# ChenFengYe/motion-latent-diffusion

Hardware: NVIDIA H100
Metric: motions/sec @ 50-step DDIM text-to-motion, batch 256 (higher is better)
Workload: dtype f16x2-split (fp32-equivalent, fp32 accumulate)

## Files before the change

include/mldb.h:

```cpp
#ifndef MLDB_H_
#define MLDB_H_

#include <stdint.h>

#ifdef __cplusplus
extern "C" {
#endif

#define MLDB_OK 0
#define MLDB_ERR_INVALID 1
#define MLDB_ERR_CUDA 2
#define MLDB_ERR_STATE 3
#define MLDB_ERR_UNSUPPORTED 4

#define MLDB_ABI_VERSION 4

typedef struct mldb_handle mldb_handle;

#define MLDB_COND_TEXT 0
#define MLDB_COND_ACTION 1
#define MLDB_ARCH_TRANS_ENC 0
#define MLDB_ARCH_TRANS_DEC 1
#define MLDB_VAE_NONE 0
#define MLDB_VAE_MLD 1
// ... 75 lines not shown

int mldb_feats2joints(mldb_handle* h, const float* feats, int32_t B, int32_t T,
                      float* joints_out, void* stream);

int mldb_sample(mldb_handle* h, const void* cond, const float* init_noise,
                const int32_t* lengths, int32_t B, int32_t S_ctx, int32_t T,
                float* latents_out, float* feats_out, float* joints_out, void* stream,
                const float* step_noise);

int mldb_sample_host(mldb_handle* h, const void* cond_host, const float* init_noise_host,
                     const int32_t* lengths_host, int32_t B, int32_t S_ctx, int32_t T,
                     float* joints_host, void* stream, const float* step_noise_host);

int mldb_comm_unique_id(void* out128 );
int mldb_comm_init(mldb_handle* h, const void* unique_id128, int32_t nranks, int32_t rank);
int mldb_comm_attach(mldb_handle* h, void* nccl_comm, int32_t nranks, int32_t rank);
int mldb_comm_info(const mldb_handle* h, int32_t* nranks, int32_t* rank);
int mldb_allgather(mldb_handle* h, const float* local, float* global, int64_t count, void* stream);
int mldb_sample_gather(mldb_handle* h, const void* cond, const float* init_noise, const int32_t* lengths,
                       int32_t B, int32_t S_ctx, int32_t T, float* joints_global, void* stream,
                       const float* step_noise);
int mldb_gather_wait(mldb_handle* h, void* stream);

int mldb_profile_op(mldb_handle* h, const char* op, int32_t B, int32_t S_ctx, int32_t iters,
                    float* avg_ms_out);

int mldb_profile_steps(mldb_handle* h, const void* cond, const float* init_noise, int32_t B, int32_t S_ctx,
                       float* ms_out);

int mldb_debug_timeline(int32_t enable, int64_t* out, int32_t cap, int32_t* count);

int mldb_debug_gemm(mldb_handle* h, const float* A, const float* W, const float* bias, const float* gamma,
                    const float* beta, const float* R, int32_t M, int32_t N, int32_t K, int32_t K1,
                    int32_t act, int32_t use_tc, int32_t split_out, float* out, void* stream);

int mldb_debug_ffn(mldb_handle* h, const float* X, const float* W1, const float* b1, const float* W2,
                   const float* b2, const float* gamma, const float* beta, int32_t M, int32_t d, int32_t ff,
                   int32_t mode, float* out, void* stream);

int mldb_debug_tail(mldb_handle* h, const float* att, const float* X, const float* Wo, const float* bo,
                    const float* gamma1, const float* beta1, const float* W1, const float* b1, const float* W2,
                    const float* b2, const float* gamma2, const float* beta2, int32_t M, int32_t d, int32_t ff,
                    int32_t mode, int32_t out_rows, float* out, void* stream);

int mldb_debug_attention(mldb_handle* h, const float* Q, const float* KV, const int32_t* lengths, int32_t kv_prefix,
                         int32_t nseq, int32_t Lq, int32_t Lk, int32_t heads, int32_t hd, int32_t mode, float* out,
                         void* stream);

int mldb_debug_attention_causal(mldb_handle* h, const float* Q, const float* KV, const int32_t* lengths,
                                int32_t kv_prefix, int32_t nseq, int32_t Lq, int32_t Lk, int32_t heads, int32_t hd,
                                int32_t mode, float* out, void* stream);

#define MLDB_TEXT_ABI_VERSION 1
#define MLDB_TEXT_HIDDEN 0
#define MLDB_TEXT_POOLED 1
typedef struct mldb_text_config {
  int32_t abi_version;
  int32_t vocab_size;
  int32_t max_positions;
  int32_t hidden;
  int32_t heads;
  int32_t layers;
  int32_t ff;
  int32_t projection_dim;
  int32_t eos_token_id;
  float   ln_eps;
} mldb_text_config;
// ... 55 lines not shown
```

mld_b200/_lib.py:

```python
from __future__ import annotations

import ctypes as C
import os

_HERE = os.path.dirname(os.path.abspath(__file__))
LIB_PATH = os.path.join(_HERE, "libmldb200.so")

MLDB_ABI_VERSION = 4
COND_TEXT, COND_ACTION = 0, 1
ARCH_TRANS_ENC, ARCH_TRANS_DEC = 0, 1
VAE_NONE, VAE_MLD, VAE_ACTOR = 0, 1, 2
SCHED_DDIM, SCHED_DDPM = 0, 1
BETA_SCHEDULES = {"scaled_linear": 0, "linear": 1, "squaredcos_cap_v2": 2}
DTYPE_F32 = 0
KSTAT_NAMES = ("gemm_tc", "gemm_ln_tc", "ffn_tc", "attn_tc", "attn_mma", "attn_simt", "gemm_simt", "ln_simt",
               "ln_unfused", "misc", "text_ln", "gru_tc")
MLDB_TEXT_ABI_VERSION = 1
TEXT_HIDDEN, TEXT_POOLED = 0, 1
MLDB_T2M_ABI_VERSION = 1
T2M_TEXT, T2M_MOVEMENT, T2M_MOTION = 1, 2, 4


class MldbConfig(C.Structure):
    _fields_ = [
# ... 22 lines not shown

class MldbT2mConfig(C.Structure):
    _fields_ = [
        ("abi_version", C.c_int32), ("parts", C.c_int32), ("dim_word", C.c_int32), ("dim_pos_ohot", C.c_int32),
        ("dim_text_hidden", C.c_int32), ("dim_coemb_hidden", C.c_int32), ("dim_pose", C.c_int32),
        ("dim_move_hidden", C.c_int32), ("dim_move_latent", C.c_int32), ("dim_motion_hidden", C.c_int32),
        ("dim_motion_latent", C.c_int32),
    ]


_P = C.c_void_p
_SIGNATURES = {
    "mldb_default_config": (None, [C.POINTER(MldbConfig)]),
    "mldb_create": (C.c_int, [C.POINTER(MldbConfig), C.c_int, C.POINTER(_P)]),
    "mldb_destroy": (None, [_P]),
    "mldb_load_tensor": (C.c_int, [_P, C.c_char_p, _P, C.POINTER(C.c_int64), C.c_int32, C.c_int32]),
    "mldb_finalize_weights": (C.c_int, [_P, _P]),
    "mldb_set_mean_std": (C.c_int, [_P, _P, _P, C.c_int32]),
    "mldb_scheduler_table": (C.c_int, [C.POINTER(MldbConfig), _P]),
    "mldb_scheduler_timesteps": (C.c_int, [C.POINTER(MldbConfig), C.c_int32, _P]),
    "mldb_scheduler_set_timesteps": (C.c_int, [_P, C.c_int32, _P]),
    "mldb_scheduler_step": (C.c_int, [_P, _P, C.c_int64, _P, _P, C.c_int64, _P, _P]),
    "mldb_denoise": (C.c_int, [_P, _P, C.c_int64, _P, _P, C.c_int32, C.c_int32, C.c_int32, _P, _P]),
    "mldb_diffusion_reverse": (C.c_int, [_P, _P, _P, _P, _P, C.c_int32, C.c_int32, C.c_int32, _P, _P]),
    "mldb_vae_decode": (C.c_int, [_P, _P, _P, C.c_int32, C.c_int32, _P, _P]),
    "mldb_vae_encode": (C.c_int, [_P, _P, _P, C.c_int32, C.c_int32, _P, _P, _P]),
    "mldb_feats2joints": (C.c_int, [_P, _P, C.c_int32, C.c_int32, _P, _P]),
    "mldb_sample": (C.c_int, [_P, _P, _P, _P, C.c_int32, C.c_int32, C.c_int32, _P, _P, _P, _P, _P]),
    "mldb_sample_host": (C.c_int, [_P, _P, _P, _P, C.c_int32, C.c_int32, C.c_int32, _P, _P, _P]),
    "mldb_profile_op": (C.c_int, [_P, C.c_char_p, C.c_int32, C.c_int32, C.c_int32, C.POINTER(C.c_float)]),
    "mldb_profile_steps": (C.c_int, [_P, _P, _P, C.c_int32, C.c_int32, _P]),
    "mldb_debug_timeline": (C.c_int, [C.c_int32, _P, C.c_int32, C.POINTER(C.c_int32)]),
    "mldb_debug_gemm": (C.c_int, [_P, _P, _P, _P, _P, _P, _P, C.c_int32, C.c_int32, C.c_int32, C.c_int32,
                                  C.c_int32, C.c_int32, C.c_int32, _P, _P]),
    "mldb_debug_ffn": (C.c_int, [_P, _P, _P, _P, _P, _P, _P, _P, C.c_int32, C.c_int32, C.c_int32, C.c_int32, _P, _P]),
    "mldb_debug_tail": (C.c_int, [_P] * 13 + [C.c_int32] * 5 + [_P, _P]),
    "mldb_debug_attention": (C.c_int, [_P, _P, _P, _P, C.c_int32, C.c_int32, C.c_int32, C.c_int32, C.c_int32, C.c_int32,
                                       C.c_int32, _P, _P]),
    "mldb_debug_attention_causal": (C.c_int, [_P, _P, _P, _P, C.c_int32, C.c_int32, C.c_int32, C.c_int32, C.c_int32,
                                              C.c_int32, C.c_int32, _P, _P]),
    "mldb_default_text_config": (None, [C.POINTER(MldbTextConfig)]),
    "mldb_text_configure": (C.c_int, [_P, C.POINTER(MldbTextConfig)]),
    "mldb_text_encode": (C.c_int, [_P, _P, C.c_int32, C.c_int32, C.c_int32, _P, _P]),
    "mldb_default_t2m_config": (None, [C.POINTER(MldbT2mConfig)]),
    "mldb_t2m_configure": (C.c_int, [_P, C.POINTER(MldbT2mConfig)]),
    "mldb_t2m_movement": (C.c_int, [_P, _P, C.c_int32, C.c_int32, C.c_int32, _P, _P]),
    "mldb_t2m_motion": (C.c_int, [_P, _P, _P, C.c_int32, C.c_int32, _P, _P]),
    "mldb_t2m_text": (C.c_int, [_P, _P, _P, _P, C.c_int32, C.c_int32, _P, _P]),
    "mldb_comm_unique_id": (C.c_int, [_P]),
    "mldb_comm_init": (C.c_int, [_P, _P, C.c_int32, C.c_int32]),
    "mldb_comm_attach": (C.c_int, [_P, _P, C.c_int32, C.c_int32]),
    "mldb_comm_info": (C.c_int, [_P, C.POINTER(C.c_int32), C.POINTER(C.c_int32)]),
    "mldb_allgather": (C.c_int, [_P, _P, _P, C.c_int64, _P]),
    "mldb_sample_gather": (C.c_int, [_P, _P, _P, _P, C.c_int32, C.c_int32, C.c_int32, _P, _P, _P]),
    "mldb_gather_wait": (C.c_int, [_P, _P]),
    "mldb_kernel_stats": (C.c_int, [_P, _P, C.c_int32]),
    "mldb_reset_kernel_stats": (C.c_int, [_P]),
    "mldb_last_error": (C.c_char_p, []),
    "mldb_abi_version": (C.c_int, []),
    "mldb_launch_count": (C.c_int64, [_P]),
    "mldb_set_option": (C.c_int, [_P, C.c_char_p, C.c_char_p]),
}

_lib = None


def lib():
# ... 40 lines not shown
```

mld_b200/csrc/engine.cu:

```cuda
#include "engine.h"

#include <math.h>
#include <stdio.h>
#include <string.h>

#include <algorithm>

#include "gemm_tc.h"

static thread_local std::string g_err;
void mldb_set_err(const std::string& s) { g_err = s; }
extern "C" const char* mldb_last_error(void) { return g_err.c_str(); }
extern "C" int mldb_abi_version(void) { return MLDB_ABI_VERSION; }

#define CK(call)                                                                      \
  do {                                                                                \
    cudaError_t e__ = (call);                                                         \
    if (e__ != cudaSuccess) {                                                         \
      char buf__[512];                                                                \
      snprintf(buf__, sizeof buf__, "%s:%d: %s failed: %s", __FILE__, __LINE__, #call, \
               cudaGetErrorString(e__));                                              \
      mldb_set_err(buf__);                                                            \
      return MLDB_ERR_CUDA;                                                           \
    }                                                                                 \
// ... 2119 lines not shown
  TRY(t2m_ready(h, MLDB_T2M_TEXT, "text"));
  const mldb_t2m_config& c = h->t2m.cfg;
  if (B < 1 || L < 1 || (int64_t)B * L > (1 << 26)) FAIL(MLDB_ERR_INVALID, "text encoder input must be [B >= 1, L >= 1, *], got B=%d L=%d", B, L);
  DeviceGuard guard(h->device);
  cudaStream_t st = (cudaStream_t)stream;
  const int W = c.dim_word, P = c.dim_pos_ohot, H = c.dim_text_hidden;
  const int Bc = t2m_chunk(h, B, gru_bytes_per_seq(L, pad64(P) + 2 * W + pad64(W) + H, H));
  for (int b0 = 0; b0 < B; b0 += Bc) {
    const int n = std::min(Bc, B - b0), M = n * L;
    ActBuf ps, xs, e;
    float* xw = nullptr;
    TRY(t2m_act(h, 0, M, pad64(P), &ps));
    TRY(t2m_slot(h, 7, (size_t)M * W * sizeof(float), (void**)&xw));
    TRY(t2m_act(h, 8, M, pad64(W), &xs));
    TRY(t2m_act(h, 2, M, H, &e));
    k_f32_to_split_pad<<<nblk((int64_t)M * ps.cols), 256, 0, st>>>(ps, pos_ohot + (int64_t)b0 * L * P, P, M, P, 1);
    kcount(h, MLDB_KSTAT_MISC);
    GemmArgs gp; gp.a1 = ps; gp.K1 = ps.cols; gp.M = M; gp.w = h->t2m.pos_emb; gp.out_f32 = xw; gp.ldc = W;
    gp.res_f32 = word_embs + (int64_t)b0 * L * W; gp.wide_n = 1;
    op_gemm(h, gp, st);
    k_f32_to_split_pad<<<nblk((int64_t)M * xs.cols), 256, 0, st>>>(xs, xw, W, M, W, 1);
    kcount(h, MLDB_KSTAT_MISC);
    GemmArgs g; g.a1 = xs; g.K1 = xs.cols; g.M = M; g.w = h->t2m.text_in; g.out = e; g.wide_n = 1;
    op_gemm(h, g, st);
    TRY(gru_forward(h, h->t2m.text_gru, e, lengths + b0, n, L, out + (int64_t)b0 * c.dim_coemb_hidden,
                    c.dim_coemb_hidden, st));
  }
  CK(cudaGetLastError());
  return check_ops(h);
}

extern "C" int mldb_debug_gemm(mldb_handle* h, const float* A, const float* W, const float* bias,
                               const float* gamma, const float* beta, const float* R, int32_t M, int32_t N,
                               int32_t K, int32_t K1, int32_t act, int32_t use_tc, int32_t split_out, float* out,
                               void* stream) {
  if (!h || !A || !W || !out || M <= 0 || N <= 0 || K <= 0) FAIL(MLDB_ERR_INVALID, "bad argument");
  DeviceGuard guard(h->device);
  cudaStream_t st = (cudaStream_t)stream;
  const size_t n_alloc0 = h->allocs.size();
  LinW w;
  TRY(pack_linear(h, W, N, K, bias, &w));
  if (K1 <= 0 || K1 >= K) K1 = K;
  ActBuf a1, a2{}, res{}, o{};
  TRY(alloc_act(h, M, K1, &a1));
  k_rows_to_split<<<nblk((int64_t)M * K1), 256, 0, st>>>(a1, A, K, M, K1, 1 << 30, 0, 0, 0, nullptr);
  if (K1 < K) {
    TRY(alloc_act(h, M, K - K1, &a2));
    k_rows_to_split<<<nblk((int64_t)M * (K - K1)), 256, 0, st>>>(a2, A + K1, K, M, K - K1, 1 << 30, 0, 0, 0, nullptr);
  }
  float *g = nullptr, *b = nullptr, *cf32 = nullptr;
  const bool saved = h->use_tc;
  h->use_tc = use_tc != 0;
  GemmArgs ga; ga.a1 = a1; ga.K1 = K1; ga.a2 = a2; ga.K2 = K - K1; ga.M = M; ga.w = w; ga.act = act; ga.wide_n = 1;
  int rc = MLDB_OK;
  if (gamma) {
    TRY(upload_f32(h, gamma, N, &g));
    TRY(upload_f32(h, beta, N, &b));
    TRY(dev_alloc(h, (void**)&cf32, (size_t)M * N * sizeof(float)));
    TRY(alloc_act(h, M, N, &o));
    if (R) {
      TRY(alloc_act(h, M, N, &res));
      k_rows_to_split<<<nblk((int64_t)M * N), 256, 0, st>>>(res, R, N, M, N, 1 << 30, 0, 0, 0, nullptr);
    }
    LnArgs l; l.res = res; l.gamma = g; l.beta = b; l.M = M; l.d = N; l.out = o;
    op_gemm_ln(h, ga, l, cf32, st);
    k_split_to_f32<<<nblk((int64_t)M * N), 256, 0, st>>>(o, out, (int64_t)M * N);
  } else if (R) {
    ga.res_f32 = R; ga.out_f32 = out; ga.ldc = N;
    op_gemm(h, ga, st);
  } else if (split_out && N % 8 == 0) {
    TRY(alloc_act(h, M, N, &o));
    ga.out = o;
    op_gemm(h, ga, st);
    k_split_to_f32<<<nblk((int64_t)M * N), 256, 0, st>>>(o, out, (int64_t)M * N);
  } else {
    ga.out_f32 = out; ga.ldc = N;
    op_gemm(h, ga, st);
  }
  h->use_tc = saved;
  cudaError_t e = cudaStreamSynchronize(st);
  if (e == cudaSuccess) e = cudaGetLastError();
  while (h->allocs.size() > n_alloc0) { cudaFree(h->allocs.back()); h->allocs.pop_back(); }
  if (e != cudaSuccess) FAIL(MLDB_ERR_CUDA, "debug gemm: %s", cudaGetErrorString(e));
  return rc;
}

extern "C" int mldb_debug_ffn(mldb_handle* h, const float* X, const float* W1, const float* b1, const float* W2,
                              const float* b2, const float* gamma, const float* beta, int32_t M, int32_t d,
                              int32_t ff, int32_t mode, float* out, void* stream) {
  if (!h || !X || !W1 || !W2 || !gamma || !beta || !out || M <= 0 || d <= 0 || ff <= 0)
    FAIL(MLDB_ERR_INVALID, "bad argument");
  DeviceGuard guard(h->device);
  cudaStream_t st = (cudaStream_t)stream;
  const size_t n_alloc0 = h->allocs.size();
  LinW l1, l2;
  LnW n;
  TRY(pack_linear(h, W1, ff, d, b1, &l1));
  TRY(pack_linear(h, W2, d, ff, b2, &l2));
  TRY(upload_f32(h, gamma, d, &n.g));
  TRY(upload_f32(h, beta, d, &n.b));
  StackWs ws;
  ws.M = M; ws.d = d; ws.ff = ff;
  ActBuf x, o;
  TRY(alloc_act(h, M, d, &x));
  TRY(alloc_act(h, M, d, &o));
  TRY(alloc_act(h, M, ff, &ws.h));
  TRY(dev_alloc(h, (void**)&ws.cf32, (size_t)M * d * sizeof(float)));
// ... 148 lines not shown
```

mld_b200/csrc/gemm_tc.cu:

```cuda
#include "gemm_tc.h"

#include <algorithm>

#include "tc_common.cuh"

namespace {
using namespace tc;

constexpr int BM = 128, BK = 64;
constexpr int NUM_THREADS = 384;
constexpr int MMA_THREADS = 256;
constexpr int CONSUMER_WARPS = 8;
constexpr int MAX_N = 1024;
constexpr int MAX_N_WIDE = 4096;

struct TcParams {
  int M, N, kblocks, kb1;
  int m_tiles, n_tiles;
  float inv_scale;
  const float* bias;
  const float* addtab;
  int act;
  __half* out_hi; __half* out_lo; int ld_out, out_col0;
  float* out_f32; int ldc;
// ... 782 lines not shown
      }
      mbar_wait(smem_u32(&bar_full[q % STAGES]), ((uint32_t)(q / STAGES)) & 1u);
      const uint32_t w = smem_u32(ring + (q % STAGES) * Cfg::STAGE_BYTES), a = sA + k * 16384;
      wg_fence();
      kblock_ss<128>(cur, a, a + 65536, w, w + Cfg::STAGE_BYTES / 2, k == 0);
      wg_commit();
      if (k == 2) {
        if (warp == 0) produce(q + 1, -1);
        if (i > 0) epilogue(prev, i - 1);
      }
      if (q > 0) {
        wg_wait<1>();
        retire(q - 1);
      }
      if (k == 0 && i > 0) acc_fence(prev);
    }
  };
  for (int i = 0; i < n; i += 2) {
    step(i, acc0, acc1);
    if (i + 1 < n) step(i + 1, acc1, acc0);
  }
  wg_wait<0>();
  retire(4 * n - 1);
  if ((n - 1) & 1) {
    acc_fence(acc1);
    epilogue(acc1, n - 1);
  } else {
    acc_fence(acc0);
    epilogue(acc0, n - 1);
  }
  tl_event(p.tl, tl_n, 42);
}

}

struct TcCtx {
  int device = 0;
  int sm_count = 132;
  int ffn_fused = 1;
  int ffn_split = 1;
};

TcCtx* tc_create(int device) {
  if (!tc::tmap_encoder()) return nullptr;
  TcCtx* c = new TcCtx();
  c->device = device;
  cudaDeviceGetAttribute(&c->sm_count, cudaDevAttrMultiProcessorCount, device);
  bool ok = true;
  auto opt_in = [&](auto kernel, int bytes) { ok = ok && smem_opt_in(kernel, bytes, "k_gemm_tc"); };
  opt_in(k_gemm_tc<256, EPI_FAST>, TileCfg<256>::SMEM_BYTES); opt_in(k_gemm_tc<128, EPI_FAST>, TileCfg<128>::SMEM_BYTES);
  opt_in(k_gemm_tc<256, EPI_FAST, ACT_GELU>, TileCfg<256>::SMEM_BYTES); opt_in(k_gemm_tc<128, EPI_FAST, ACT_GELU>, TileCfg<128>::SMEM_BYTES);
  opt_in(k_gemm_tc<256, EPI_GENERIC>, TileCfg<256>::SMEM_BYTES); opt_in(k_gemm_tc<128, EPI_GENERIC>, TileCfg<128>::SMEM_BYTES);
  opt_in(k_gemm_tc<256, EPI_FAST, ACT_QUICKGELU>, TileCfg<256>::SMEM_BYTES);
  opt_in(k_gemm_tc<128, EPI_FAST, ACT_QUICKGELU>, TileCfg<128>::SMEM_BYTES);
  opt_in(k_gemm_tc<256, EPI_RES>, TileCfg<256>::SMEM_BYTES); opt_in(k_gemm_tc<128, EPI_RES>, TileCfg<128>::SMEM_BYTES);
  opt_in(k_gemm_tc<256, EPI_LN>, TileCfg<256>::SMEM_BYTES);
  opt_in(k_gemm_tc<256, EPI_FAST, ACT_LEAKY>, TileCfg<256>::SMEM_BYTES); opt_in(k_gemm_tc<128, EPI_FAST, ACT_LEAKY>, TileCfg<128>::SMEM_BYTES);
  opt_in(k_gemm_tc<256, EPI_F32>, TileCfg<256>::SMEM_BYTES); opt_in(k_gemm_tc<128, EPI_F32>, TileCfg<128>::SMEM_BYTES);
  opt_in(k_gemm_tc<256, EPI_F32, ACT_LEAKY>, TileCfg<256>::SMEM_BYTES); opt_in(k_gemm_tc<128, EPI_F32, ACT_LEAKY>, TileCfg<128>::SMEM_BYTES);
  opt_in(k_ffn_tc, FfnCfg::SMEM_BYTES);
  opt_in(k_proj_tc<ACT_NONE>, ProjCfg::SMEM_BYTES); opt_in(k_proj_tc<ACT_GELU>, ProjCfg::SMEM_BYTES);
  opt_in(k_proj_tc<ACT_QUICKGELU>, ProjCfg::SMEM_BYTES); opt_in(k_proj_tc<ACT_LEAKY>, ProjCfg::SMEM_BYTES);
  if (!ok) {
    delete c;
    return nullptr;
  }
  return c;
}
void tc_destroy(TcCtx* c) { delete c; }

static int pick_bn(const GemmArgs& g) { return (g.w.N % 256 == 0) ? 256 : 128; }

bool tc_gemm_supported(const TcCtx* c, const GemmArgs& g) {
  if (!c) return false;
  if (g.a_kind != A_SPLIT || g.M < 1 || g.w.N > (g.wide_n ? MAX_N_WIDE : MAX_N)) return false;
  if (g.K1 <= 0 || g.K1 % BK || g.K2 % BK || g.a1.cols != g.K1) return false;
  if (g.K2 > 0 && g.a2.cols != g.K2) return false;
  if (g.w.K != g.K1 + g.K2) return false;
  if (((uintptr_t)g.a1.hi & 15) || ((uintptr_t)g.w.w & 15)) return false;
  if (g.out.hi && ((g.out.cols % 8) || (g.out_col0 % 8))) return false;
  if (g.res_f32 && (!g.out_f32 || g.out.hi || g.act != ACT_NONE || g.addtab || g.zero_lengths || g.in_group < g.M ||
                    g.out_group != 0 || g.out_off != 0 || (g.w.N % 2) || (g.ldc % 2) || ((uintptr_t)g.out_f32 & 7) ||
                    ((uintptr_t)g.res_f32 & 7)))
    return false;
  return true;
}

bool tc_gemm_ln_supported(const TcCtx* c, const GemmArgs& g, const LnArgs& l) {
  if (!tc_gemm_supported(c, g)) return false;
  if (g.w.N != 256 || l.d != 256 || g.act != ACT_NONE) return false;
  if (l.in_group != 0 || l.c != nullptr || l.out_f32 != nullptr || !l.out.hi) return false;
  if (l.out.cols != 256 || (l.res.hi && l.res.cols != 256)) return false;
  if (l.gamma2 || l.rowvec) return false;
  if (g.addtab || g.zero_lengths || g.in_group < g.M || g.out_group != 0 || g.out_off != 0) return false;
  return true;
}

static void fill_params(const GemmArgs& g, const LnArgs* ln, int bn, TcParams* out) {
  TcParams p{};
  p.M = g.M; p.N = g.w.N; p.kblocks = g.w.K / BK; p.kb1 = g.K1 / BK;
  p.inv_scale = g.w.inv_scale; p.bias = g.w.bias; p.addtab = g.addtab; p.act = g.act;
  p.in_group = g.in_group; p.out_group = g.out_group; p.out_off = g.out_off; p.zero_lengths = g.zero_lengths;
  if (ln) {
    p.out_hi = ln->out.hi; p.out_lo = ln->out.lo(); p.ld_out = ln->out.cols; p.out_col0 = 0;
    p.res_hi = ln->res.hi; p.res_lo = ln->res.hi ? ln->res.lo() : nullptr; p.ld_res = ln->res.cols;
    p.gamma = ln->gamma; p.beta = ln->beta;
  } else {
    p.out_hi = g.out.hi; p.out_lo = g.out.hi ? g.out.lo() : nullptr; p.ld_out = g.out.cols; p.out_col0 = g.out_col0;
    p.out_f32 = g.out_f32; p.ldc = g.ldc; p.res_f32 = g.res_f32;
  }
  p.m_tiles = (g.M + BM - 1) / BM;
  p.n_tiles = (g.w.N + bn - 1) / bn;
  p.tl = tc::mldb_timeline_buffer();
  *out = p;
}

static bool tc_proj(TcCtx* c, const GemmArgs& g, cudaStream_t st) {
  CUtensorMap mAh, mAl, mWh, mWl;
  const bool ok = make_map(&mAh, g.a1.hi, g.M, g.K1, BM) && make_map(&mAl, g.a1.lo(), g.M, g.K1, BM) &&
                  make_map(&mWh, g.w.w, g.w.N, g.w.K, ProjCfg::CHUNK) &&
                  make_map(&mWl, g.w.w + g.w.plane_stride, g.w.N, g.w.K, ProjCfg::CHUNK);
  if (!ok) return false;
  ProjParams p{};
  p.M = g.M; p.n_chunks = g.w.N / ProjCfg::CHUNK; p.items = (g.M + BM - 1) / BM * p.n_chunks;
  p.inv_scale = g.w.inv_scale; p.bias = g.w.bias;
  p.out_hi = g.out.hi; p.out_lo = g.out.lo(); p.ld_out = g.out.cols; p.out_col0 = g.out_col0;
  p.tl = tc::mldb_timeline_buffer();
  const dim3 grid(p.items < c->sm_count ? p.items : c->sm_count);
  switch (g.act) {
    case ACT_GELU: launch_pdl(k_proj_tc<ACT_GELU>, grid, dim3(MMA_THREADS), ProjCfg::SMEM_BYTES, st, mAh, mAl, mWh, mWl, p); break;
    case ACT_QUICKGELU: launch_pdl(k_proj_tc<ACT_QUICKGELU>, grid, dim3(MMA_THREADS), ProjCfg::SMEM_BYTES, st, mAh, mAl, mWh, mWl, p); break;
    case ACT_LEAKY: launch_pdl(k_proj_tc<ACT_LEAKY>, grid, dim3(MMA_THREADS), ProjCfg::SMEM_BYTES, st, mAh, mAl, mWh, mWl, p); break;
    default: launch_pdl(k_proj_tc<ACT_NONE>, grid, dim3(MMA_THREADS), ProjCfg::SMEM_BYTES, st, mAh, mAl, mWh, mWl, p); break;
  }
  return true;
}

bool tc_gemm(TcCtx* c, const GemmArgs& g, const LnArgs* ln, cudaStream_t st) {
  const int bn = ln ? 256 : pick_bn(g);
  const bool fast = !ln && g.out.hi && !g.out_f32 && !g.addtab && !g.zero_lengths && g.in_group >= g.M &&
                    g.out_group == 0 && g.out_off == 0 && g.w.N % bn == 0 && g.w.bias != nullptr &&
                    (g.act == ACT_NONE || g.act == ACT_GELU || g.act == ACT_QUICKGELU || g.act == ACT_LEAKY);
  if (fast && g.K1 == 256 && g.K2 == 0 && ((uintptr_t)g.out.hi & 15) == 0 && ((uintptr_t)g.out.lo() & 15) == 0)
    return tc_proj(c, g, st);
  CUtensorMap mA1h, mA1l, mA2h, mA2l, mWh, mWl;
  bool ok = make_map(&mA1h, g.a1.hi, g.M, g.K1, BM) && make_map(&mA1l, g.a1.lo(), g.M, g.K1, BM);
  if (g.K2 > 0) ok = ok && make_map(&mA2h, g.a2.hi, g.M, g.K2, BM) && make_map(&mA2l, g.a2.lo(), g.M, g.K2, BM);
  else { mA2h = mA1h; mA2l = mA1l; }
  ok = ok && make_map(&mWh, g.w.w, g.w.N, g.w.K, bn) && make_map(&mWl, g.w.w + g.w.plane_stride, g.w.N, g.w.K, bn);
  if (!ok) return false;
  TcParams p;
  fill_params(g, ln, bn, &p);
  const bool f32 = !ln && g.vec_f32 && !g.out.hi && g.out_f32 && !g.res_f32 && !g.addtab && !g.zero_lengths &&
                   g.in_group >= g.M && g.out_group == 0 && g.out_off == 0 && g.w.N % 2 == 0 && g.ldc % 2 == 0 &&
                   ((uintptr_t)g.out_f32 & 7) == 0 && (g.act == ACT_NONE || g.act == ACT_LEAKY);
  const int ntiles = p.m_tiles * p.n_tiles;
  dim3 grid(ntiles < c->sm_count ? ntiles : c->sm_count);
#define MLDB_LAUNCH(BN_, ...)                                                                                      \
  launch_pdl(k_gemm_tc<BN_, __VA_ARGS__>, grid, dim3(NUM_THREADS), TileCfg<BN_>::SMEM_BYTES, st, mA1h, mA1l, mA2h, \
             mA2l, mWh, mWl, p)
#define MLDB_LAUNCH_SHAPE(...)                                                       \
  do {                                                                               \
    if (bn == 256) MLDB_LAUNCH(256, __VA_ARGS__); else MLDB_LAUNCH(128, __VA_ARGS__); \
  } while (0)
  if (ln)                             MLDB_LAUNCH(256, EPI_LN);
  else if (g.res_f32)                 MLDB_LAUNCH_SHAPE(EPI_RES);
  else if (fast && g.act == ACT_GELU) MLDB_LAUNCH_SHAPE(EPI_FAST, ACT_GELU);
  else if (fast && g.act == ACT_QUICKGELU) MLDB_LAUNCH_SHAPE(EPI_FAST, ACT_QUICKGELU);
  else if (fast && g.act == ACT_LEAKY) MLDB_LAUNCH_SHAPE(EPI_FAST, ACT_LEAKY);
  else if (f32 && g.act == ACT_LEAKY) MLDB_LAUNCH_SHAPE(EPI_F32, ACT_LEAKY);
  else if (f32)                       MLDB_LAUNCH_SHAPE(EPI_F32);
  else if (fast)                      MLDB_LAUNCH_SHAPE(EPI_FAST);
  else                                MLDB_LAUNCH_SHAPE(EPI_GENERIC);
#undef MLDB_LAUNCH_SHAPE
#undef MLDB_LAUNCH
  return true;
}

int tc_set_ffn_split(TcCtx* c, int on) {
  if (!c) return 0;
  const int old = c->ffn_split;
  c->ffn_split = on;
  return old;
}
int tc_set_ffn_fused(TcCtx* c, int on) {
  if (!c) return 0;
  const int old = c->ffn_fused;
  c->ffn_fused = on;
  return old;
}
static bool planes_aligned16(const ActBuf& b) { return ((uintptr_t)b.hi & 15) == 0 && ((uintptr_t)b.lo() & 15) == 0; }

bool tc_ffn_supported(const TcCtx* c, const GemmArgs& g1, const GemmArgs& g2, const LnArgs& l2) {
  if (!c || !c->ffn_fused) return false;
  if (!tc_gemm_supported(c, g1) || !tc_gemm_ln_supported(c, g2, l2)) return false;
  if (g1.K1 != 256 || g1.K2 > 0 || g2.K2 > 0 || g1.M != g2.M) return false;
  if (g1.w.N % FfnCfg::CHUNK || g1.w.N > MAX_N || g1.w.N != g2.K1) return false;
  if (g1.act != ACT_GELU || g1.out_f32 || g1.addtab || g1.zero_lengths) return false;
  if (g1.in_group < g1.M || g1.out_group != 0 || g1.out_off != 0) return false;
  if (l2.res.hi != g1.a1.hi || l2.res.plane_stride != g1.a1.plane_stride) return false;
  if (!planes_aligned16(g1.a1) || !planes_aligned16(l2.out)) return false;
  return true;
}
bool tc_tail_supported(const TcCtx* c, const GemmArgs& go, const LnArgs& l1, const GemmArgs& g1, const GemmArgs& g2,
                       const LnArgs& l2) {
  if (!tc_gemm_ln_supported(c, go, l1) || !tc_ffn_supported(c, g1, g2, l2)) return false;
  if (go.K1 != 256 || go.K2 > 0 || go.M != g1.M || !l1.res.hi) return false;
  if (g1.a1.hi != l1.out.hi || g1.a1.plane_stride != l1.out.plane_stride) return false;
  return planes_aligned16(go.a1) && planes_aligned16(l1.res);
}

static bool launch_ffn(TcCtx* c, const GemmArgs* go, const LnArgs* l1, const GemmArgs& g1, const GemmArgs& g2,
                       const LnArgs& l2, float* scratch, int* flags, cudaStream_t st) {
  CUtensorMap mXh, mXl, mW1h, mW1l, mW2h, mW2l, mAh, mAl, mWoh, mWol, mYh, mYl;
  const int M = g1.M, m_tiles = (M + BM - 1) / BM;
  const ActBuf x = go ? l1->res : g1.a1;
  bool ok = make_map(&mXh, x.hi, M, 256, BM) && make_map(&mXl, x.lo(), M, 256, BM) &&
            make_map(&mW1h, g1.w.w, g1.w.N, g1.w.K, FfnCfg::CHUNK) &&
            make_map(&mW1l, g1.w.w + g1.w.plane_stride, g1.w.N, g1.w.K, FfnCfg::CHUNK) &&
            make_map(&mW2h, g2.w.w, g2.w.N, g2.w.K, 256) &&
            make_map(&mW2l, g2.w.w + g2.w.plane_stride, g2.w.N, g2.w.K, 256) &&
            make_map(&mYh, l2.out.hi, M, 256, 64) && make_map(&mYl, l2.out.lo(), M, 256, 64);
  if (go) {
    ok = ok && make_map(&mAh, go->a1.hi, M, 256, BM) && make_map(&mAl, go->a1.lo(), M, 256, BM) &&
         make_map(&mWoh, go->w.w, go->w.N, go->w.K, 256) && make_map(&mWol, go->w.w + go->w.plane_stride, go->w.N, go->w.K, 256);
// ... 32 lines not shown
```

mld_b200/engine.py:

```python
from __future__ import annotations

import ctypes as C
from typing import Dict, Optional, Sequence

import torch

from . import _lib
from ._lib import MldbConfig, check


def _ptr(t: Optional[torch.Tensor]):
    return None if t is None else C.c_void_p(t.data_ptr())


def _f32c(t: torch.Tensor, device) -> torch.Tensor:
    return t.to(device=device, dtype=torch.float32).contiguous()


class Engine:

    def __init__(self, cfg: MldbConfig, device: int | torch.device = 0):
        self._h = None
        self.lib = _lib.lib()
        if not torch.cuda.is_available():
# ... 19 lines not shown
            t = v.detach().to(dtype=torch.float32).contiguous()
            shape = (C.c_int64 * t.dim())(*t.shape)
            check(self.lib.mldb_load_tensor(self._h, (prefix + k).encode(), _ptr(t), shape, t.dim(),
                                            _lib.DTYPE_F32), f"mldb_load_tensor({prefix + k})")

    def finalize(self):
        check(self.lib.mldb_finalize_weights(self._h, None), "mldb_finalize_weights")

    def set_mean_std(self, mean: torch.Tensor, std: torch.Tensor):
        m = mean.detach().float().contiguous().cpu()
        s = std.detach().float().contiguous().cpu()
        check(self.lib.mldb_set_mean_std(self._h, _ptr(m), _ptr(s), m.numel()), "mldb_set_mean_std")

    def set_option(self, name: str, value: str):
        check(self.lib.mldb_set_option(self._h, name.encode(), value.encode()), "mldb_set_option")

    def profile_op(self, op: str, B: int, S_ctx: int, iters: int = 20) -> float:
        ms = C.c_float()
        check(self.lib.mldb_profile_op(self._h, op.encode(), B, S_ctx, iters, C.byref(ms)), "mldb_profile_op")
        return float(ms.value)

    def profile_steps(self, cond: torch.Tensor, init_noise: torch.Tensor):
        c, z0 = self._cond(cond), _f32c(init_noise, self.device)
        B = z0.shape[0]
        self._check_latent(z0, B, "init_noise")
        self._check_cond(c, 2 * B if self.cfg_on else B)
        S = c.shape[1] if c.dim() == 3 else 1
        n = 0 if self.timesteps is None else len(self.timesteps)
        ms = (C.c_float * n)()
        check(self.lib.mldb_profile_steps(self._h, _ptr(c), _ptr(z0), B, S, ms), "mldb_profile_steps")
        return [float(v) for v in ms]

    def debug_gemm(self, A, W, bias=None, gamma=None, beta=None, R=None, K1=0, act=0, use_tc=True, split_out=False,
                   in_place=False):
        A = _f32c(A, self.device)
        Wc = W.detach().float().contiguous().cpu()
        host = [None if t is None else t.detach().float().contiguous().cpu() for t in (bias, gamma, beta)]
        Rd = None if R is None else _f32c(R, self.device)
        M, K = A.shape
        N = Wc.shape[0]
        out = torch.empty((M, N), dtype=torch.float32, device=self.device)
        if in_place:
            if Rd is None or gamma is not None:
                raise ValueError("in_place needs R and no gamma (the residual-add epilogue)")
            out = Rd = Rd.clone()
        check(self.lib.mldb_debug_gemm(self._h, _ptr(A), _ptr(Wc), _ptr(host[0]), _ptr(host[1]), _ptr(host[2]),
                                       _ptr(Rd), M, N, K, K1, act, int(use_tc), int(split_out), _ptr(out), self._stream()),
              "mldb_debug_gemm")
        return out

    def debug_ffn(self, X, W1, b1, W2, b2, gamma, beta, mode=2):
        X = _f32c(X, self.device)
        host = [t.detach().float().contiguous().cpu() for t in (W1, b1, W2, b2, gamma, beta)]
        M, d = X.shape
        ff = host[0].shape[0]
        out = torch.empty((M, d), dtype=torch.float32, device=self.device)
        check(self.lib.mldb_debug_ffn(self._h, _ptr(X), *[_ptr(t) for t in host], M, d, ff, int(mode), _ptr(out),
                                      self._stream()), "mldb_debug_ffn")
        return out

    def debug_tail(self, att, X, Wo, bo, g1, be1, W1, b1, W2, b2, g2, be2, mode=2, pad=None):
        att, X = _f32c(att, self.device), _f32c(X, self.device)
        host = [None if t is None else t.detach().float().contiguous().cpu()
                for t in (Wo, bo, g1, be1, W1, b1, W2, b2, g2, be2)]
        M, d = X.shape
        ff = host[4].shape[0]
        out = torch.empty((M, d), dtype=torch.float32, device=self.device)
        if pad is not None:
            out = torch.cat([out, _f32c(pad, self.device)]).contiguous()
        check(self.lib.mldb_debug_tail(self._h, _ptr(att), _ptr(X), *[_ptr(t) for t in host], M, d, ff, int(mode),
                                       out.shape[0], _ptr(out), self._stream()), "mldb_debug_tail")
        return out

    def debug_attention(self, q, nseq, Lq, heads, lengths=None, mode=2, kv=None, Lk=None, kv_prefix=0,
                        causal=False):
        q = _f32c(q, self.device)
        kvd = None if kv is None else _f32c(kv, self.device)
        d = q.shape[1] // 3 if kv is None else q.shape[1]
        Lk = Lq if Lk is None else Lk
        if q.shape[0] != nseq * Lq or (kvd is not None and tuple(kvd.shape) != (nseq * Lk, 2 * d)):
# ... 372 lines not shown
```

Baseline: 856.1.

## Add persistent TMA/WGMMA kernel for K=256 GEMM with fused LayerNorm epilogue

```diff
diff --git a/include/mldb.h b/include/mldb.h
--- a/include/mldb.h
+++ b/include/mldb.h
@@ -131,7 +131,7 @@
 
 int mldb_debug_gemm(mldb_handle* h, const float* A, const float* W, const float* bias, const float* gamma,
                     const float* beta, const float* R, int32_t M, int32_t N, int32_t K, int32_t K1,
-                    int32_t act, int32_t use_tc, int32_t split_out, float* out, void* stream);
+                    int32_t act, int32_t use_tc, int32_t split_out, int32_t out_rows, float* out, void* stream);
 
 int mldb_debug_ffn(mldb_handle* h, const float* X, const float* W1, const float* b1, const float* W2,
                    const float* b2, const float* gamma, const float* beta, int32_t M, int32_t d, int32_t ff,
diff --git a/mld_b200/_lib.py b/mld_b200/_lib.py
--- a/mld_b200/_lib.py
+++ b/mld_b200/_lib.py
@@ -78,7 +78,7 @@
     "mldb_profile_steps": (C.c_int, [_P, _P, _P, C.c_int32, C.c_int32, _P]),
     "mldb_debug_timeline": (C.c_int, [C.c_int32, _P, C.c_int32, C.POINTER(C.c_int32)]),
     "mldb_debug_gemm": (C.c_int, [_P, _P, _P, _P, _P, _P, _P, C.c_int32, C.c_int32, C.c_int32, C.c_int32,
-                                  C.c_int32, C.c_int32, C.c_int32, _P, _P]),
+                                  C.c_int32, C.c_int32, C.c_int32, C.c_int32, _P, _P]),
     "mldb_debug_ffn": (C.c_int, [_P, _P, _P, _P, _P, _P, _P, _P, C.c_int32, C.c_int32, C.c_int32, C.c_int32, _P, _P]),
     "mldb_debug_tail": (C.c_int, [_P] * 13 + [C.c_int32] * 5 + [_P, _P]),
     "mldb_debug_attention": (C.c_int, [_P, _P, _P, _P, C.c_int32, C.c_int32, C.c_int32, C.c_int32, C.c_int32, C.c_int32,
diff --git a/mld_b200/csrc/engine.cu b/mld_b200/csrc/engine.cu
--- a/mld_b200/csrc/engine.cu
+++ b/mld_b200/csrc/engine.cu
@@ -2175,9 +2175,9 @@
 
 extern "C" int mldb_debug_gemm(mldb_handle* h, const float* A, const float* W, const float* bias,
                                const float* gamma, const float* beta, const float* R, int32_t M, int32_t N,
-                               int32_t K, int32_t K1, int32_t act, int32_t use_tc, int32_t split_out, float* out,
-                               void* stream) {
-  if (!h || !A || !W || !out || M <= 0 || N <= 0 || K <= 0) FAIL(MLDB_ERR_INVALID, "bad argument");
+                               int32_t K, int32_t K1, int32_t act, int32_t use_tc, int32_t split_out,
+                               int32_t out_rows, float* out, void* stream) {
+  if (!h || !A || !W || !out || M <= 0 || N <= 0 || K <= 0 || out_rows < M) FAIL(MLDB_ERR_INVALID, "bad argument");
   DeviceGuard guard(h->device);
   cudaStream_t st = (cudaStream_t)stream;
   const size_t n_alloc0 = h->allocs.size();
@@ -2196,26 +2196,32 @@
   h->use_tc = use_tc != 0;
   GemmArgs ga; ga.a1 = a1; ga.K1 = K1; ga.a2 = a2; ga.K2 = K - K1; ga.M = M; ga.w = w; ga.act = act; ga.wide_n = 1;
   int rc = MLDB_OK;
+  auto split_out_buf = [&]() -> int {
+    TRY(alloc_act(h, out_rows, N, &o));
+    if (out_rows > M)
+      k_rows_to_split<<<nblk((int64_t)out_rows * N), 256, 0, st>>>(o, out, N, out_rows, N, 1 << 30, 0, 0, 0, nullptr);
+    return MLDB_OK;
+  };
   if (gamma) {
     TRY(upload_f32(h, gamma, N, &g));
     TRY(upload_f32(h, beta, N, &b));
     TRY(dev_alloc(h, (void**)&cf32, (size_t)M * N * sizeof(float)));
-    TRY(alloc_act(h, M, N, &o));
+    TRY(split_out_buf());
     if (R) {
       TRY(alloc_act(h, M, N, &res));
       k_rows_to_split<<<nblk((int64_t)M * N), 256, 0, st>>>(res, R, N, M, N, 1 << 30, 0, 0, 0, nullptr);
     }
     LnArgs l; l.res = res; l.gamma = g; l.beta = b; l.M = M; l.d = N; l.out = o;
     op_gemm_ln(h, ga, l, cf32, st);
-    k_split_to_f32<<<nblk((int64_t)M * N), 256, 0, st>>>(o, out, (int64_t)M * N);
+    k_split_to_f32<<<nblk((int64_t)out_rows * N), 256, 0, st>>>(o, out, (int64_t)out_rows * N);
   } else if (R) {
     ga.res_f32 = R; ga.out_f32 = out; ga.ldc = N;
     op_gemm(h, ga, st);
   } else if (split_out && N % 8 == 0) {
-    TRY(alloc_act(h, M, N, &o));
+    TRY(split_out_buf());
     ga.out = o;
     op_gemm(h, ga, st);
-    k_split_to_f32<<<nblk((int64_t)M * N), 256, 0, st>>>(o, out, (int64_t)M * N);
+    k_split_to_f32<<<nblk((int64_t)out_rows * N), 256, 0, st>>>(o, out, (int64_t)out_rows * N);
   } else {
     ga.out_f32 = out; ga.ldc = N;
     op_gemm(h, ga, st);
diff --git a/mld_b200/csrc/gemm_tc.cu b/mld_b200/csrc/gemm_tc.cu
--- a/mld_b200/csrc/gemm_tc.cu
+++ b/mld_b200/csrc/gemm_tc.cu
@@ -838,6 +838,181 @@
   tl_event(p.tl, tl_n, 42);
 }
 
+struct OutLnParams {
+  int M, m_tiles;
+  float inv_scale;
+  const float* bias; const float* gamma; const float* beta;
+  const __half* res_hi; const __half* res_lo;
+  __half* out_hi; __half* out_lo;
+  long long* tl;
+};
+
+__global__ void __launch_bounds__(MMA_THREADS, 1)
+k_outln_tc(const __grid_constant__ CUtensorMap tmAh, const __grid_constant__ CUtensorMap tmAl,
+           const __grid_constant__ CUtensorMap tmWh, const __grid_constant__ CUtensorMap tmWl,
+           const __grid_constant__ CUtensorMap tmRh, const __grid_constant__ CUtensorMap tmRl, const OutLnParams p) {
+  using Cfg = ProjCfg;
+  constexpr int STAGES = Cfg::STAGES;
+  extern __shared__ uint8_t smem_raw[];
+  uint8_t* smem = smem_raw + smem_pad1024(smem_raw);
+  uint8_t* ring = smem + Cfg::A_BYTES;
+  uint64_t* bar_full = reinterpret_cast<uint64_t*>(ring + STAGES * Cfg::STAGE_BYTES);
+  uint64_t* bar_empty = bar_full + STAGES;
+  uint64_t* bar_afull = bar_empty + STAGES;
+  uint64_t* bar_aempty = bar_afull + 4;
+
+  const int warp = __shfl_sync(0xffffffffu, (int)(threadIdx.x >> 5), 0), lane = threadIdx.x & 31;
+  int tl_n = 0;
+  tl_event(p.tl, tl_n, 40);
+  const int n = (p.m_tiles - (int)blockIdx.x + (int)gridDim.x - 1) / (int)gridDim.x;
+  auto tile_m0 = [&](int j) { return ((int)blockIdx.x + j * (int)gridDim.x) * BM; };
+
+  if (threadIdx.x == 0) {
+    for (int s = 0; s < STAGES; ++s) {
+      mbar_init(smem_u32(&bar_full[s]), 1);
+      mbar_init(smem_u32(&bar_empty[s]), CONSUMER_WARPS);
+    }
+    for (int k = 0; k < 4; ++k) {
+      mbar_init(smem_u32(&bar_afull[k]), 1);
+      mbar_init(smem_u32(&bar_aempty[k]), CONSUMER_WARPS);
+    }
+    asm volatile("fence.mbarrier_init.release.cluster;" ::: "memory");
+    tma_prefetch_desc(&tmAh); tma_prefetch_desc(&tmAl); tma_prefetch_desc(&tmWh); tma_prefetch_desc(&tmWl);
+    if (p.res_hi) { tma_prefetch_desc(&tmRh); tma_prefetch_desc(&tmRl); }
+  }
+  pdl_trigger();
+  __syncthreads();
+  pdl_wait();
+  tl_event(p.tl, tl_n, 41);
+
+  int q_next = 0, a_next = 0;
+  auto load_w = [&](int q) {
+    if (elect_one()) {
+      const int c = q & 1, k = (q >> 1) & 3;
+      const uint32_t full = smem_u32(&bar_full[q % STAGES]);
+      const uint32_t dst = smem_u32(ring + (q % STAGES) * Cfg::STAGE_BYTES);
+      mbar_expect_tx(full, Cfg::STAGE_BYTES);
+      tma_load_2d(dst, &tmWh, full, k * BK, c * Cfg::CHUNK);
+      tma_load_2d(dst + Cfg::STAGE_BYTES / 2, &tmWl, full, k * BK, c * Cfg::CHUNK);
+    }
+    __syncwarp();
+  };
+  auto load_a = [&](int a) {
+    if (elect_one()) {
+      const int j = a >> 2, k = a & 3, m0 = tile_m0(j);
+      const uint32_t full = smem_u32(&bar_afull[k]);
+      mbar_expect_tx(full, 2 * BM * 128);
+      tma_load_2d(smem_u32(smem + k * 16384), &tmAh, full, k * BK, m0);
+      tma_load_2d(smem_u32(smem + 65536 + k * 16384), &tmAl, full, k * BK, m0);
+      if (k == 0) {
+        if (p.res_hi)
+          for (int k2 = 0; k2 < 4; ++k2) { tma_prefetch_2d(&tmRh, k2 * BK, m0); tma_prefetch_2d(&tmRl, k2 * BK, m0); }
+        if (j + 1 < n)
+          for (int k2 = 0; k2 < 4; ++k2) { tma_prefetch_2d(&tmAh, k2 * BK, tile_m0(j + 1)); tma_prefetch_2d(&tmAl, k2 * BK, tile_m0(j + 1)); }
+      }
+    }
+    __syncwarp();
+  };
+  auto produce = [&](int need_w, int need_a) {
+    ring_produce(a_next, 4 * n, need_a, bar_aempty, 4, load_a);
+    ring_produce(q_next, 8 * n, need_w, bar_empty, STAGES, load_w);
+  };
+
+  const int cw = warp >> 2;
+  const int cp = 2 * (lane & 3), l = lane & 3;
+  const uint32_t sA = smem_u32(smem) + cw * (64 * 128);
+  float acc[128];
+  auto retire = [&](int q) {
+    if (lane == 0) {
+      mbar_arrive(smem_u32(&bar_empty[q % STAGES]));
+      if (q & 1) mbar_arrive(smem_u32(&bar_aempty[(q >> 1) & 3]));
+    }
+  };
+  for (int j = 0; j < n; ++j) {
+    tl_event(p.tl, tl_n, 70, j);
+#pragma unroll
+    for (int k = 0; k < 4; ++k) {
+#pragma unroll
+      for (int c = 0; c < 2; ++c) {
+        const int q = 8 * j + 2 * k + c;
+        if (warp == 0) produce(q, 4 * j + k);
+        if (c == 0) {
+          mbar_wait(smem_u32(&bar_afull[k]), (uint32_t)j & 1u);
+          if (k == 0) tl_event(p.tl, tl_n, 71, j);
+        }
+        mbar_wait(smem_u32(&bar_full[q % STAGES]), ((uint32_t)(q / STAGES)) & 1u);
+        const uint32_t w = smem_u32(ring + (q % STAGES) * Cfg::STAGE_BYTES), a = sA + k * 16384;
+        wg_fence();
+        kblock_ss<128>(*reinterpret_cast<float(*)[64]>(acc + 64 * c), a, a + 65536, w, w + Cfg::STAGE_BYTES / 2, k == 0);
+        wg_commit();
+        if (k + c > 0) {
+          wg_wait<1>();
+          retire(q - 1);
+        }
+      }
+    }
+    wg_wait<0>();
+    retire(8 * j + 7);
+    acc_fence(acc);
+    if (warp == 0) produce(8 * j + 10, 4 * j + 7);
+    tl_event(p.tl, tl_n, 72, j);
+    const int r_lo = tile_m0(j) + cw * 64 + (warp & 3) * 16 + (lane >> 2);
+    const bool ok0 = r_lo < p.M, ok1 = r_lo + 8 < p.M;
+    const int64_t o0 = (int64_t)r_lo * 256 + 8 * l, o1 = o0 + 8 * 256;
+    uint32_t v[4][4];
+    uint4 nxt[4];
+    auto ld = [&](int jb) {
+      const uint4 z = make_uint4(0u, 0u, 0u, 0u);
+      nxt[0] = ok0 ? *reinterpret_cast<const uint4*>(p.res_hi + o0 + 32 * jb) : z;
+      nxt[1] = ok0 ? *reinterpret_cast<const uint4*>(p.res_lo + o0 + 32 * jb) : z;
+      nxt[2] = ok1 ? *reinterpret_cast<const uint4*>(p.res_hi + o1 + 32 * jb) : z;
+      nxt[3] = ok1 ? *reinterpret_cast<const uint4*>(p.res_lo + o1 + 32 * jb) : z;
+    };
+    ln_rows(acc, p.inv_scale, p.bias, p.gamma, p.beta, cp,
+            [&](int jj, float (&x)[4]) {
+              if (p.res_hi) {
+                const int g = jj & 3;
+                if (jj == 0) ld(0);
+                if (g == 0) {
+#pragma unroll
+                  for (int r = 0; r < 4; ++r) {
+                    v[r][0] = nxt[r].x; v[r][1] = nxt[r].y; v[r][2] = nxt[r].z; v[r][3] = nxt[r].w;
+                    quad_transpose(v[r], l);
+                  }
+                  if (jj < 28) ld((jj >> 2) + 1);
+                }
+#pragma unroll
+                for (int h = 0; h < 2; ++h) {
+                  const float2 hi = __half22float2(*reinterpret_cast<const __half2*>(&v[2 * h][g]));
+                  const float2 lo = __half22float2(*reinterpret_cast<const __half2*>(&v[2 * h + 1][g]));
+                  x[2 * h] = (x[2 * h] + hi.x) + lo.x; x[2 * h + 1] = (x[2 * h + 1] + hi.y) + lo.y;
+                }
+              }
+              if (jj == 31) tl_event(p.tl, tl_n, 73, j);
+            },
+            [&](int jj, const float (&y)[4]) {
+              const int g = jj & 3;
+              split2(y[0], y[1], v[0][g], v[1][g]);
+              split2(y[2], y[3], v[2][g], v[3][g]);
+              if (g == 3) {
+#pragma unroll
+                for (int r = 0; r < 4; ++r) quad_transpose(v[r], l);
+                const int64_t o = 8 * (jj - 3);
+                if (ok0) {
+                  *reinterpret_cast<uint4*>(p.out_hi + o0 + o) = make_uint4(v[0][0], v[0][1], v[0][2], v[0][3]);
+                  *reinterpret_cast<uint4*>(p.out_lo + o0 + o) = make_uint4(v[1][0], v[1][1], v[1][2], v[1][3]);
+                }
+                if (ok1) {
+                  *reinterpret_cast<uint4*>(p.out_hi + o1 + o) = make_uint4(v[2][0], v[2][1], v[2][2], v[2][3]);
+                  *reinterpret_cast<uint4*>(p.out_lo + o1 + o) = make_uint4(v[3][0], v[3][1], v[3][2], v[3][3]);
+                }
+              }
+            });
+    tl_event(p.tl, tl_n, 74, j);
+  }
+  tl_event(p.tl, tl_n, 42);
+}
+
 }
 
 struct TcCtx {
@@ -867,6 +1042,7 @@
   opt_in(k_ffn_tc, FfnCfg::SMEM_BYTES);
   opt_in(k_proj_tc<ACT_NONE>, ProjCfg::SMEM_BYTES); opt_in(k_proj_tc<ACT_GELU>, ProjCfg::SMEM_BYTES);
   opt_in(k_proj_tc<ACT_QUICKGELU>, ProjCfg::SMEM_BYTES); opt_in(k_proj_tc<ACT_LEAKY>, ProjCfg::SMEM_BYTES);
+  opt_in(k_outln_tc, ProjCfg::SMEM_BYTES);
   if (!ok) {
     delete c;
     return nullptr;
@@ -920,6 +1096,8 @@
   p.tl = tc::mldb_timeline_buffer();
   *out = p;
 }
+
+static bool planes_aligned16(const ActBuf& b) { return ((uintptr_t)b.hi & 15) == 0 && ((uintptr_t)b.lo() & 15) == 0; }
 
 static bool tc_proj(TcCtx* c, const GemmArgs& g, cudaStream_t st) {
   CUtensorMap mAh, mAl, mWh, mWl;
@@ -942,6 +1120,25 @@
   return true;
 }
 
+static bool tc_outln(TcCtx* c, const GemmArgs& g, const LnArgs& l, cudaStream_t st) {
+  CUtensorMap mAh, mAl, mWh, mWl, mRh, mRl;
+  bool ok = make_map(&mAh, g.a1.hi, g.M, g.K1, BM) && make_map(&mAl, g.a1.lo(), g.M, g.K1, BM) &&
+            make_map(&mWh, g.w.w, g.w.N, g.w.K, ProjCfg::CHUNK) &&
+            make_map(&mWl, g.w.w + g.w.plane_stride, g.w.N, g.w.K, ProjCfg::CHUNK);
+  if (l.res.hi) ok = ok && make_map(&mRh, l.res.hi, g.M, 256, BM) && make_map(&mRl, l.res.lo(), g.M, 256, BM);
+  else { mRh = mAh; mRl = mAl; }
+  if (!ok) return false;
+  OutLnParams p{};
+  p.M = g.M; p.m_tiles = (g.M + BM - 1) / BM;
+  p.inv_scale = g.w.inv_scale; p.bias = g.w.bias; p.gamma = l.gamma; p.beta = l.beta;
+  p.res_hi = l.res.hi; p.res_lo = l.res.hi ? l.res.lo() : nullptr;
+  p.out_hi = l.out.hi; p.out_lo = l.out.lo();
+  p.tl = tc::mldb_timeline_buffer();
+  const dim3 grid(p.m_tiles < c->sm_count ? p.m_tiles : c->sm_count);
+  launch_pdl(k_outln_tc, grid, dim3(MMA_THREADS), ProjCfg::SMEM_BYTES, st, mAh, mAl, mWh, mWl, mRh, mRl, p);
+  return true;
+}
+
 bool tc_gemm(TcCtx* c, const GemmArgs& g, const LnArgs* ln, cudaStream_t st) {
   const int bn = ln ? 256 : pick_bn(g);
   const bool fast = !ln && g.out.hi && !g.out_f32 && !g.addtab && !g.zero_lengths && g.in_group >= g.M &&
@@ -949,6 +1146,8 @@
                     (g.act == ACT_NONE || g.act == ACT_GELU || g.act == ACT_QUICKGELU || g.act == ACT_LEAKY);
   if (fast && g.K1 == 256 && g.K2 == 0 && ((uintptr_t)g.out.hi & 15) == 0 && ((uintptr_t)g.out.lo() & 15) == 0)
     return tc_proj(c, g, st);
+  if (ln && g.K1 == 256 && g.K2 == 0 && planes_aligned16(ln->out) && (!ln->res.hi || planes_aligned16(ln->res)))
+    return tc_outln(c, g, *ln, st);
   CUtensorMap mA1h, mA1l, mA2h, mA2l, mWh, mWl;
   bool ok = make_map(&mA1h, g.a1.hi, g.M, g.K1, BM) && make_map(&mA1l, g.a1.lo(), g.M, g.K1, BM);
   if (g.K2 > 0) ok = ok && make_map(&mA2h, g.a2.hi, g.M, g.K2, BM) && make_map(&mA2l, g.a2.lo(), g.M, g.K2, BM);
@@ -995,8 +1194,6 @@
   c->ffn_fused = on;
   return old;
 }
-static bool planes_aligned16(const ActBuf& b) { return ((uintptr_t)b.hi & 15) == 0 && ((uintptr_t)b.lo() & 15) == 0; }
-
 bool tc_ffn_supported(const TcCtx* c, const GemmArgs& g1, const GemmArgs& g2, const LnArgs& l2) {
   if (!c || !c->ffn_fused) return false;
   if (!tc_gemm_supported(c, g1) || !tc_gemm_ln_supported(c, g2, l2)) return false;
diff --git a/mld_b200/engine.py b/mld_b200/engine.py
--- a/mld_b200/engine.py
+++ b/mld_b200/engine.py
@@ -75,7 +75,7 @@
         return [float(v) for v in ms]
 
     def debug_gemm(self, A, W, bias=None, gamma=None, beta=None, R=None, K1=0, act=0, use_tc=True, split_out=False,
-                   in_place=False):
+                   in_place=False, pad=None):
         A = _f32c(A, self.device)
         Wc = W.detach().float().contiguous().cpu()
         host = [None if t is None else t.detach().float().contiguous().cpu() for t in (bias, gamma, beta)]
@@ -87,8 +87,13 @@
             if Rd is None or gamma is not None:
                 raise ValueError("in_place needs R and no gamma (the residual-add epilogue)")
             out = Rd = Rd.clone()
+        if pad is not None:
+            if gamma is None and not split_out:
+                raise ValueError("pad needs a split16 output (gamma or split_out)")
+            out = torch.cat([out, _f32c(pad, self.device)]).contiguous()
         check(self.lib.mldb_debug_gemm(self._h, _ptr(A), _ptr(Wc), _ptr(host[0]), _ptr(host[1]), _ptr(host[2]),
-                                       _ptr(Rd), M, N, K, K1, act, int(use_tc), int(split_out), _ptr(out), self._stream()),
+                                       _ptr(Rd), M, N, K, K1, act, int(use_tc), int(split_out), out.shape[0],
+                                       _ptr(out), self._stream()),
               "mldb_debug_gemm")
         return out
 
```

After: 876.6, median of 6. +2.4%, better.
